# JuliaReinforcementLearning/ReinforcementLearning.jl

Measured on NVIDIA H100. Metric: env-steps/sec at 65536 CartPole envs (full PPO iteration: rollout T=32 + GAE + 4 epochs x 4 minibatches), higher is better.
Workload: dtype f32

## Files before the change

### include/b200rl.h

```cpp
#ifndef B200RL_H
#define B200RL_H

#include <stddef.h>
#include <stdint.h>

#ifdef __cplusplus
extern "C" {
#endif

typedef enum {
    B200RL_OK = 0,
    B200RL_ERR_INVALID = -1,
    B200RL_ERR_CUDA = -2,
    B200RL_ERR_UNSUPPORTED = -3,
    B200RL_ERR_ACTION = -4,
    B200RL_ERR_NCCL = -5,
    B200RL_ERR_OOM = -6
} b200rl_status;

typedef struct b200rl_ctx b200rl_ctx;
typedef struct b200rl_env b200rl_env;
typedef struct b200rl_traj b200rl_traj;
typedef struct b200rl_net b200rl_net;

// ... 68 lines not shown
int b200rl_env_reset(b200rl_env* env, int force_all);
int b200rl_env_step(b200rl_env* env, const void* actions, int actions_on_device, int auto_reset);
int b200rl_env_step_random(b200rl_env* env, int auto_reset);
int b200rl_env_get(b200rl_env* env, int field, void* host_dst, size_t bytes);
int b200rl_env_set(b200rl_env* env, int field, const void* host_src, size_t bytes);
int b200rl_env_ptr(b200rl_env* env, int field, void** dptr_out);
int b200rl_env_check(b200rl_env* env);
int b200rl_env_episode_stats(b200rl_env* env, double* out4, int reset_after);

int b200rl_gae_f32(b200rl_ctx* ctx, float* adv, const float* rewards, const float* values,
                   const uint8_t* terminal, float gamma, float lambda, int64_t R, int64_t C,
                   int dims, int on_device);
int b200rl_gae_f64(b200rl_ctx* ctx, double* adv, const double* rewards, const double* values,
                   const uint8_t* terminal, double gamma, double lambda, int64_t R, int64_t C,
                   int dims, int on_device);
int b200rl_discount_rewards_f32(b200rl_ctx* ctx, float* out, const float* rewards,
                                const uint8_t* terminal, const float* init, float gamma,
                                int64_t R, int64_t C, int dims, int on_device);
int b200rl_discount_rewards_f64(b200rl_ctx* ctx, double* out, const double* rewards,
                                const uint8_t* terminal, const double* init, double gamma,
                                int64_t R, int64_t C, int dims, int on_device);
int b200rl_discount_rewards_reduced_f32(b200rl_ctx* ctx, float* out, const float* rewards,
                                        const uint8_t* terminal, const float* init, float gamma,
                                        int64_t R, int64_t C, int dims, int on_device);
int b200rl_discount_rewards_reduced_f64(b200rl_ctx* ctx, double* out, const double* rewards,
                                        const uint8_t* terminal, const double* init, double gamma,
                                        int64_t R, int64_t C, int dims, int on_device);

int b200rl_traj_create(b200rl_ctx* ctx, int ns, int64_t lanes, int64_t capacity, int prioritized, float default_priority,
                       const uint64_t* sampler_rng, int64_t batch_size, b200rl_traj** out);
int b200rl_traj_destroy(b200rl_traj* traj);
int b200rl_traj_length(b200rl_traj* traj, int64_t* frames_out);
int b200rl_traj_lane_lengths(b200rl_traj* traj, int64_t* lengths_out);
int b200rl_traj_n_sampleable(b200rl_traj* traj, int64_t* out);
int b200rl_traj_push_state(b200rl_traj* traj, const float* obs, int on_device);
int b200rl_traj_push_episode_start(b200rl_traj* traj, const float* obs, int on_device, int mode);
int b200rl_traj_push(b200rl_traj* traj, const int32_t* action, const float* reward, const uint8_t* terminal, const float* next_obs,
                     int on_device);
int b200rl_traj_push_env(b200rl_traj* traj, b200rl_env* env, int first_state_only);
int b200rl_traj_field_bytes(b200rl_traj* traj, int field, size_t* bytes_out);
int b200rl_traj_get(b200rl_traj* traj, int field, void* host_dst, size_t bytes);
int b200rl_traj_set(b200rl_traj* traj, int field, const void* host_src, size_t bytes);
int b200rl_traj_sample(b200rl_traj* traj, float beta);
int b200rl_traj_set_nstep(b200rl_traj* traj, int32_t n, float gamma);
int b200rl_traj_batch_get(b200rl_traj* traj, int field, void* host_dst, size_t bytes);
int b200rl_traj_update_priority(b200rl_traj* traj, const float* priority, int on_device);
int b200rl_traj_total_priority(b200rl_traj* traj, float* out);

typedef struct { int32_t n_in, hidden, act, n_out, kind; } b200rl_net_desc;
int b200rl_net_nparams(const b200rl_net_desc* desc, int64_t* out);
int b200rl_net_create(b200rl_ctx* ctx, const b200rl_net_desc* desc, const float* params_host, b200rl_net** out);
int b200rl_net_destroy(b200rl_net* net);
int b200rl_net_configure_optimizer(b200rl_net* net, float lr, float beta1, float beta2, float eps, float max_grad_norm);
int b200rl_net_get(b200rl_net* net, int which, float* host_dst, int64_t count);
int b200rl_net_set(b200rl_net* net, int which, const float* host_src, int64_t count);
int b200rl_net_ptr(b200rl_net* net, int which, void** dptr_out);
int b200rl_net_get_step(b200rl_net* net, int64_t* out);
int b200rl_net_set_step(b200rl_net* net, int64_t step);
int b200rl_net_target_sync(b200rl_net* net, float rho);
int b200rl_net_act(b200rl_net* net, const float* obs, int64_t n, uint64_t* rng_dev, void* action_out, float* logp_out, float* value_out,
                   float* heads_out, int on_device);
int b200rl_net_values(b200rl_net* net, const float* obs, int64_t n, float* out, int use_target, int on_device);
int b200rl_net_q_act(b200rl_net* net, const float* obs_dev, int64_t n, uint64_t* rng_dev, float epsilon, int32_t* action_out_dev);
typedef struct {
    double eps_stable, eps_init;
    int64_t warmup_steps, decay_steps;
    int64_t step;
    int32_t kind;
    int32_t is_break_tie;
    double beta;
} b200rl_explorer;
int b200rl_net_q_explore(b200rl_net* net, const float* obs_dev, int64_t n, uint64_t* rng_dev, const b200rl_explorer* explorer,
                         int32_t* action_out_dev);
int b200rl_net_act_greedy(b200rl_net* net, const float* obs, int64_t n, void* action_out, int on_device);

typedef struct { int32_t mode, n_steps, max_episodes; } b200rl_eval_config;
int b200rl_evaluate(b200rl_net* net, b200rl_env* env, const b200rl_eval_config* cfg, uint64_t* policy_rng_dev,
                    float* returns_out, int32_t* lengths_out, int32_t* counts_out, int on_device);
int b200rl_evaluate_explore(b200rl_net* net, b200rl_env* env, int32_t n_steps, int32_t max_episodes, b200rl_explorer* ex,
                            uint64_t* explorer_rng_dev, float* returns_out, int32_t* lengths_out, int32_t* counts_out, int on_device);

typedef struct {
    float gamma, lambda, clip_range, max_grad_norm, w_actor, w_critic, w_entropy;
    float lr, beta1, beta2, eps;
    float min_sigma, max_sigma;
    int32_t normalize_advantage, n_epochs, n_microbatches, update_freq;
    int32_t algo;
} b200rl_onpolicy_config;
typedef struct b200rl_onpolicy b200rl_onpolicy;
int b200rl_net_ac_step(b200rl_net* net, const b200rl_onpolicy_config* cfg, const float* states, const void* actions,
                       const float* logp_old, const float* adv, const float* ret, int64_t total, const int32_t* idx, int64_t batch,
                       float adv_mean, float adv_inv_std, int apply_update, float* losses_out);
int b200rl_onpolicy_create(b200rl_ctx* ctx, b200rl_net* net, b200rl_env* env, const b200rl_onpolicy_config* cfg,
                           const uint64_t* policy_rng, b200rl_onpolicy** out);
int b200rl_onpolicy_destroy(b200rl_onpolicy* agent);
int b200rl_onpolicy_plan(b200rl_onpolicy* agent, void* actions_host);
int b200rl_onpolicy_act(b200rl_onpolicy* agent);
int b200rl_onpolicy_push(b200rl_onpolicy* agent);
int b200rl_onpolicy_collect(b200rl_onpolicy* agent, int n_steps);
int b200rl_onpolicy_fill(b200rl_onpolicy* agent, int* t_out, int* T_out);
int b200rl_onpolicy_update(b200rl_onpolicy* agent, const int32_t* perm_host, float* stats_host);
int b200rl_onpolicy_iterate(b200rl_onpolicy* agent, int n_iters, float* stats_host);
int b200rl_onpolicy_graph_active(b200rl_onpolicy* agent, int* out);
int b200rl_onpolicy_get(b200rl_onpolicy* agent, int field, void* host_dst, size_t bytes);
int b200rl_onpolicy_set(b200rl_onpolicy* agent, int field, const void* host_src, size_t bytes);
int b200rl_onpolicy_export_state(b200rl_onpolicy* agent, int64_t* counters3_out);
// ... 37 lines not shown
```

### reinforcementlearning.jl_b200/_lib.py

```python
import ctypes as C
import os

import numpy as np

HERE = os.path.dirname(os.path.abspath(__file__))
SO_PATH = os.environ.get("B200RL_LIB") or os.path.join(HERE, "libb200rl.so")

OK = 0
ERR_INVALID, ERR_CUDA, ERR_UNSUPPORTED, ERR_ACTION, ERR_NCCL, ERR_OOM = -1, -2, -3, -4, -5, -6

ENV_CARTPOLE, ENV_PENDULUM, ENV_MOUNTAINCAR, ENV_CARTPOLE_CONTINUOUS, ENV_MOUNTAINCAR_CONTINUOUS, ENV_ACROBOT = 0, 1, 2, 3, 4, 5
F32, F64 = 0, 1
FIELD_STATE, FIELD_OBS, FIELD_REWARD, FIELD_TERMINAL, FIELD_T, FIELD_RNG, FIELD_FLAGS, FIELD_ACTION, FIELD_EPISODE_RETURN, FIELD_EPISODE_STATS = range(10)


class B200RLError(RuntimeError):
    def __init__(self, status, msg):
        super().__init__(f"b200rl status {status}: {msg}")
        self.status = status


class CartPoleParams(C.Structure):
    _fields_ = [(n, C.c_double) for n in ("gravity", "masscart", "masspole", "totalmass", "halflength", "polemasslength",
                                          "forcemag", "dt", "thetathreshold", "xthreshold")] + [("max_steps", C.c_int64)]
# ... 56 lines not shown
    "b200rl_timer_stop_ms": (_i32, [_vp, C.POINTER(_f32)]),
    "b200rl_timer_record": (_i32, [_vp, _i32]),
    "b200rl_timer_elapsed_ms": (_i32, [_vp, _i32, _i32, C.POINTER(_f32)]),
    "b200rl_debug_phase_slots": (_i32, [_vp, _i32]),
    "b200rl_malloc": (_i32, [_vp, _sz, _pp]),
    "b200rl_free": (_i32, [_vp, _vp]),
    "b200rl_host_alloc": (_i32, [_vp, _sz, _pp]),
    "b200rl_host_free": (_i32, [_vp, _vp]),
    "b200rl_memcpy_h2d": (_i32, [_vp, _vp, _vp, _sz, _i32]),
    "b200rl_memcpy_d2h": (_i32, [_vp, _vp, _vp, _sz, _i32]),
    "b200rl_memset": (_i32, [_vp, _vp, _i32, _sz]),
    "b200rl_flush_l2": (_i32, [_vp]),
    "b200rl_launch_count": (_i32, [_vp, C.POINTER(_u64)]),
    "b200rl_env_create": (_i32, [_vp, _i32, _i32, _i64, _vp, _vp, _pp]),
    "b200rl_env_destroy": (_i32, [_vp]),
    "b200rl_env_set_max_timeout": (_i32, [_vp, _i64]),
    "b200rl_env_copy": (_i32, [_vp, _pp]),
    "b200rl_env_seed": (_i32, [_vp, _vp]),
    "b200rl_env_reset": (_i32, [_vp, _i32]),
    "b200rl_env_step": (_i32, [_vp, _vp, _i32, _i32]),
    "b200rl_env_step_random": (_i32, [_vp, _i32]),
    "b200rl_env_get": (_i32, [_vp, _i32, _vp, _sz]),
    "b200rl_env_set": (_i32, [_vp, _i32, _vp, _sz]),
    "b200rl_env_ptr": (_i32, [_vp, _i32, _pp]),
    "b200rl_env_check": (_i32, [_vp]),
    "b200rl_env_episode_stats": (_i32, [_vp, _vp, _i32]),
    "b200rl_gae_f32": (_i32, [_vp, _vp, _vp, _vp, _vp, _f32, _f32, _i64, _i64, _i32, _i32]),
    "b200rl_gae_f64": (_i32, [_vp, _vp, _vp, _vp, _vp, _f64, _f64, _i64, _i64, _i32, _i32]),
    "b200rl_discount_rewards_f32": (_i32, [_vp, _vp, _vp, _vp, _vp, _f32, _i64, _i64, _i32, _i32]),
    "b200rl_discount_rewards_f64": (_i32, [_vp, _vp, _vp, _vp, _vp, _f64, _i64, _i64, _i32, _i32]),
    "b200rl_discount_rewards_reduced_f32": (_i32, [_vp, _vp, _vp, _vp, _vp, _f32, _i64, _i64, _i32, _i32]),
    "b200rl_discount_rewards_reduced_f64": (_i32, [_vp, _vp, _vp, _vp, _vp, _f64, _i64, _i64, _i32, _i32]),
    "b200rl_traj_create": (_i32, [_vp, _i32, _i64, _i64, _i32, _f32, _vp, _i64, _pp]),
    "b200rl_traj_destroy": (_i32, [_vp]),
    "b200rl_traj_length": (_i32, [_vp, C.POINTER(_i64)]),
    "b200rl_traj_lane_lengths": (_i32, [_vp, _vp]),
    "b200rl_traj_n_sampleable": (_i32, [_vp, C.POINTER(_i64)]),
    "b200rl_traj_push_episode_start": (_i32, [_vp, _vp, _i32, _i32]),
    "b200rl_traj_field_bytes": (_i32, [_vp, _i32, C.POINTER(_sz)]),
    "b200rl_traj_get": (_i32, [_vp, _i32, _vp, _sz]),
    "b200rl_traj_set": (_i32, [_vp, _i32, _vp, _sz]),
    "b200rl_traj_push_state": (_i32, [_vp, _vp, _i32]),
    "b200rl_traj_push": (_i32, [_vp, _vp, _vp, _vp, _vp, _i32]),
    "b200rl_traj_push_env": (_i32, [_vp, _vp, _i32]),
    "b200rl_traj_sample": (_i32, [_vp, _f32]),
    "b200rl_traj_set_nstep": (_i32, [_vp, _i32, _f32]),
    "b200rl_traj_batch_get": (_i32, [_vp, _i32, _vp, _sz]),
    "b200rl_traj_update_priority": (_i32, [_vp, _vp, _i32]),
    "b200rl_traj_total_priority": (_i32, [_vp, C.POINTER(_f32)]),
    "b200rl_net_nparams": (_i32, [_vp, C.POINTER(_i64)]),
    "b200rl_net_create": (_i32, [_vp, _vp, _vp, _pp]),
    "b200rl_net_destroy": (_i32, [_vp]),
    "b200rl_net_configure_optimizer": (_i32, [_vp, _f32, _f32, _f32, _f32, _f32]),
    "b200rl_net_get": (_i32, [_vp, _i32, _vp, _i64]),
    "b200rl_net_set": (_i32, [_vp, _i32, _vp, _i64]),
    "b200rl_net_ptr": (_i32, [_vp, _i32, _pp]),
    "b200rl_net_get_step": (_i32, [_vp, C.POINTER(_i64)]),
    "b200rl_net_set_step": (_i32, [_vp, _i64]),
    "b200rl_net_target_sync": (_i32, [_vp, _f32]),
    "b200rl_net_act": (_i32, [_vp, _vp, _i64, _vp, _vp, _vp, _vp, _vp, _i32]),
    "b200rl_net_values": (_i32, [_vp, _vp, _i64, _vp, _i32, _i32]),
    "b200rl_net_q_act": (_i32, [_vp, _vp, _i64, _vp, _f32, _vp]),
    "b200rl_net_q_explore": (_i32, [_vp, _vp, _i64, _vp, _vp, _vp]),
    "b200rl_net_act_greedy": (_i32, [_vp, _vp, _i64, _vp, _i32]),
    "b200rl_evaluate": (_i32, [_vp, _vp, _vp, _vp, _vp, _vp, _vp, _i32]),
    "b200rl_evaluate_explore": (_i32, [_vp, _vp, _i32, _i32, _vp, _vp, _vp, _vp, _vp, _i32]),
    "b200rl_net_ac_step": (_i32, [_vp, _vp, _vp, _vp, _vp, _vp, _vp, _i64, _vp, _i64, _f32, _f32, _i32, _vp]),
    "b200rl_onpolicy_create": (_i32, [_vp, _vp, _vp, _vp, _vp, _pp]),
    "b200rl_onpolicy_destroy": (_i32, [_vp]),
    "b200rl_onpolicy_plan": (_i32, [_vp, _vp]),
    "b200rl_onpolicy_act": (_i32, [_vp]),
    "b200rl_onpolicy_push": (_i32, [_vp]),
    "b200rl_onpolicy_collect": (_i32, [_vp, _i32]),
    "b200rl_onpolicy_fill": (_i32, [_vp, C.POINTER(_i32), C.POINTER(_i32)]),
    "b200rl_onpolicy_update": (_i32, [_vp, _vp, _vp]),
    "b200rl_onpolicy_iterate": (_i32, [_vp, _i32, _vp]),
    "b200rl_onpolicy_graph_active": (_i32, [_vp, C.POINTER(_i32)]),
    "b200rl_onpolicy_get": (_i32, [_vp, _i32, _vp, _sz]),
    "b200rl_onpolicy_set": (_i32, [_vp, _i32, _vp, _sz]),
    "b200rl_onpolicy_export_state": (_i32, [_vp, _vp]),
    "b200rl_onpolicy_import_state": (_i32, [_vp, _vp]),
    "b200rl_onpolicy_time_kernel": (_i32, [_vp, _i32, _i32, C.POINTER(_f32)]),
    "b200rl_dqn_update": (_i32, [_vp, _vp, _vp, _vp]),
    "b200rl_dqn_last_td": (_i32, [_vp, _vp, _vp, _i64]),
    "b200rl_replay_create": (_i32, [_vp, _vp, _vp, _vp, _vp, _pp]),
    "b200rl_replay_run": (_i32, [_vp, _vp, _vp, _vp, _i64, _vp]),
    "b200rl_replay_graph_active": (_i32, [_vp, C.POINTER(_i32)]),
    "b200rl_replay_destroy": (_i32, [_vp]),
    "b200rl_set_tensor_cores": (_i32, [_i32]),
    "b200rl_set_fused_step": (_i32, [_i32]),
    "b200rl_comm_unique_id": (_i32, [_vp]),
    "b200rl_comm_init": (_i32, [_vp, _i32, _i32, _vp]),
    "b200rl_comm_allreduce_f32": (_i32, [_vp, _vp, _i64]),
    "b200rl_comm_p2p_export": (_i32, [_vp, _vp, _pp]),
    "b200rl_comm_p2p_open": (_i32, [_vp, _vp, _pp]),
    "b200rl_comm_p2p_attach": (_i32, [_vp, _vp]),
    "b200rl_ctx_pci_bus_id": (_i32, [_vp, _vp, _i32]),
    "b200rl_comm_p2p_set_exclusive": (_i32, [_vp, _i32]),
}

_LIB = None


def load():
    global _LIB
    if _LIB is not None:
# ... 113 lines not shown
```

### reinforcementlearning.jl_b200/csrc/algo.cu

```cuda
#include <map>

#include "greedy.cuh"
#include "internal.h"
#include "nn.cuh"
#include "replay_schedule.h"
#include "ring.cuh"

static void* env_field(b200rl_env* e, int f) { void* p = nullptr; b200rl_env_ptr(e, f, &p); return p; }

namespace {
__global__ void clamp_copy_kernel(float* __restrict__ dst, const float* __restrict__ src, int64_t n, float lo, float hi) {
    int64_t i = (int64_t)blockIdx.x * blockDim.x + threadIdx.x;
    if (i < n) dst[i] = fminf(fmaxf(src[i], lo), hi);
}
__global__ void greedy_select_kernel(const float* __restrict__ heads, MlpDesc d, int64_t n, int clamp, float lo, float hi,
                                     uint32_t* __restrict__ out) {
    int64_t i = (int64_t)blockIdx.x * blockDim.x + threadIdx.x;
    if (i >= n) return;
    float z[kOutMax];
#pragma unroll
    for (int o = 0; o < kOutMax; ++o) z[o] = o < d.nout ? heads[(int64_t)d.nout * i + o] : 0.f;
    uint32_t a = greedy::greedy_action(d, z);
    if (clamp) a = __float_as_uint(fminf(fmaxf(__uint_as_float(a), lo), hi));
    out[i] = a;
// ... 267 lines not shown
extern "C" {

int b200rl_net_nparams(const b200rl_net_desc* d, int64_t* out) {
    MlpDesc a, c;
    TRY(make_descs(d, &a, &c));
    REQUIRE(out, B200RL_ERR_INVALID, "null out");
    *out = is_q_kind(d->kind) ? a.nparams() : a.nparams() + c.nparams();
    return B200RL_OK;
}

int b200rl_net_destroy(b200rl_net* n) {
    if (!n) return B200RL_OK;
    cudaSetDevice(n->ctx->device);
    cudaStreamSynchronize(n->ctx->stream);
    cudaFree(n->params); cudaFree(n->grad); cudaFree(n->m); cudaFree(n->v); cudaFree(n->beta_t); cudaFree(n->target);
    cudaFree(n->partial); cudaFree(n->loss_partial); cudaFree(n->loss4); cudaFree(n->gnorm); cudaFree(n->cta_sumsq); cudaFree(n->counters);
    delete n;
    return B200RL_OK;
}

int b200rl_net_create(b200rl_ctx* ctx, const b200rl_net_desc* d, const float* params_host, b200rl_net** out) {
    TRY(ctx_bind(ctx));
    REQUIRE(out && params_host, B200RL_ERR_INVALID, "null argument");
    b200rl_net* n = new b200rl_net();
    memset(n, 0, sizeof *n);
    n->ctx = ctx; n->kind = d ? d->kind : 0;
    int s = make_descs(d, &n->actor, &n->critic);
    if (s != B200RL_OK) { delete n; return s; }
    n->np = is_q_kind(n->kind) ? n->actor.nparams() : n->actor.nparams() + n->critic.nparams();
    n->lr = 1e-3f; n->b1 = 0.9f; n->b2 = 0.999f; n->eps = 1e-8f; n->max_grad_norm = 0.5f;
    size_t bytes = (size_t)n->np * sizeof(float);
    n->n_partials = is_q_kind(n->kind) ? nn_dqn_max_partials(ctx, n->actor.H) : nn_grid_ctas(ctx, n->actor.H);
    int n_loss_rows = 2 * (n->n_partials > ctx->sm_count ? n->n_partials : ctx->sm_count);
#define NET_TRY(x) CUDA_TRY_OR(x, b200rl_net_destroy(n))
    NET_TRY(cudaMalloc(&n->params, bytes)); NET_TRY(cudaMalloc(&n->grad, bytes)); NET_TRY(cudaMalloc(&n->m, bytes)); NET_TRY(cudaMalloc(&n->v, bytes));
    NET_TRY(cudaMalloc(&n->beta_t, 2 * sizeof(float)));
    if (is_q_kind(n->kind)) NET_TRY(cudaMalloc(&n->target, bytes));
    NET_TRY(cudaMalloc(&n->partial, (size_t)n->n_partials * bytes));
    NET_TRY(cudaMalloc(&n->loss_partial, (size_t)n_loss_rows * 4 * sizeof(float)));
    NET_TRY(cudaMalloc(&n->loss4, 4 * sizeof(float))); NET_TRY(cudaMalloc(&n->gnorm, sizeof(float)));
    NET_TRY(cudaMalloc(&n->cta_sumsq, 256 * sizeof(double))); NET_TRY(cudaMalloc(&n->counters, 4 * sizeof(unsigned int)));
    NET_TRY(cudaMemsetAsync(n->counters, 0, 4 * sizeof(unsigned int), ctx->stream));
    NET_TRY(cudaMemcpyAsync(n->params, params_host, bytes, cudaMemcpyHostToDevice, ctx->stream));
    if (is_q_kind(n->kind)) NET_TRY(cudaMemcpyAsync(n->target, params_host, bytes, cudaMemcpyHostToDevice, ctx->stream));
    NET_TRY(cudaMemsetAsync(n->grad, 0, bytes, ctx->stream)); NET_TRY(cudaMemsetAsync(n->m, 0, bytes, ctx->stream));
    NET_TRY(cudaMemsetAsync(n->v, 0, bytes, ctx->stream));
    NET_TRY(cudaMemsetAsync(n->partial, 0, (size_t)n->n_partials * bytes, ctx->stream));
    NET_TRY(cudaMemsetAsync(n->loss_partial, 0, (size_t)n_loss_rows * 4 * sizeof(float), ctx->stream));
    float bt[2] = {n->b1, n->b2};
    NET_TRY(cudaMemcpyAsync(n->beta_t, bt, sizeof bt, cudaMemcpyHostToDevice, ctx->stream));
    NET_TRY(cudaStreamSynchronize(ctx->stream));
#undef NET_TRY
    *out = n;
    return B200RL_OK;
}

int b200rl_net_configure_optimizer(b200rl_net* n, float lr, float beta1, float beta2, float eps, float max_grad_norm) {
    REQUIRE(n, B200RL_ERR_INVALID, "null net");
    TRY(ctx_bind(n->ctx));
    n->lr = lr; n->b1 = beta1; n->b2 = beta2; n->eps = eps; n->max_grad_norm = max_grad_norm;
    if (n->n_updates == 0) {
        float bt[2] = {beta1, beta2};
        CUDA_TRY(cudaMemcpyAsync(n->beta_t, bt, sizeof bt, cudaMemcpyHostToDevice, n->ctx->stream));
        CUDA_TRY(cudaStreamSynchronize(n->ctx->stream));
    }
    return B200RL_OK;
}

static int net_buf(b200rl_net* n, int which, float** p, int64_t* len) {
    switch (which) {
        case 0: *p = n->params; *len = n->np; return B200RL_OK;
        case 1: *p = n->grad; *len = n->np; return B200RL_OK;
        case 2: *p = n->m; *len = n->np; return B200RL_OK;
        case 3: *p = n->v; *len = n->np; return B200RL_OK;
        case 4: *p = n->beta_t; *len = 2; return B200RL_OK;
        case 5: REQUIRE(n->target, B200RL_ERR_INVALID, "no target network"); *p = n->target; *len = n->np; return B200RL_OK;
    }
    REQUIRE(false, B200RL_ERR_INVALID, "unknown buffer id");
}
int b200rl_net_get(b200rl_net* n, int which, float* host_dst, int64_t count) {
    REQUIRE(n && host_dst, B200RL_ERR_INVALID, "null argument");
    TRY(ctx_bind(n->ctx));
    float* p; int64_t len;
    TRY(net_buf(n, which, &p, &len));
    REQUIRE(count >= len, B200RL_ERR_INVALID, "destination too small");
    CUDA_TRY(cudaMemcpyAsync(host_dst, p, (size_t)len * 4, cudaMemcpyDeviceToHost, n->ctx->stream));
    CUDA_TRY(cudaStreamSynchronize(n->ctx->stream));
    return B200RL_OK;
}
int b200rl_net_set(b200rl_net* n, int which, const float* host_src, int64_t count) {
    REQUIRE(n && host_src, B200RL_ERR_INVALID, "null argument");
    TRY(ctx_bind(n->ctx));
    float* p; int64_t len;
    TRY(net_buf(n, which, &p, &len));
    REQUIRE(count >= len, B200RL_ERR_INVALID, "source too small");
    CUDA_TRY(cudaMemcpyAsync(p, host_src, (size_t)len * 4, cudaMemcpyHostToDevice, n->ctx->stream));
    CUDA_TRY(cudaStreamSynchronize(n->ctx->stream));
    return B200RL_OK;
}
int b200rl_net_ptr(b200rl_net* n, int which, void** dptr_out) {
    REQUIRE(n && dptr_out, B200RL_ERR_INVALID, "null argument");
    float* p; int64_t len;
    TRY(net_buf(n, which, &p, &len));
    *dptr_out = p;
    return B200RL_OK;
}
// ... 907 lines not shown
```

### reinforcementlearning.jl_b200/csrc/nn_tc.cu

```cuda
#include "nn.cuh"
#include "perm.cuh"
#include "policy.cuh"
#include "tc_fwd.cuh"
#include "tc_split.h"
#include "wgmma.cuh"

namespace {

using tcfwd::G_F;
using tcfwd::GW_S;
using tcfwd::WIMG_BYTES;
using tcfwd::split2;
using tcfwd::wimg_off;
constexpr int TM = tcfwd::TM;
constexpr int H = tcfwd::H;
constexpr float kScaleW = tcfwd::kScale;

constexpr int NT7 = 512;
constexpr int kMaxStage = 10;
constexpr int GF_T = 128;
constexpr int GS_T = 16 * GF_T;
constexpr int FIMG = 8 * GS_T;
constexpr float kScaleH = 64.0f, kScaleX = 64.0f;
constexpr int kNo = 2;

struct SmemBwd {
    static_assert(FIMG % 128 == 0 && WIMG_BYTES % 128 == 0 && (2 * GS_T) % 16 == 0, "operand images must stay 128-byte aligned");
    alignas(128) uint8_t FP_full[FIMG];
    alignas(128) uint8_t FP_lo[FIMG];
    alignas(128) uint8_t FH_lo[FIMG];
    alignas(128) uint8_t FH_full[FIMG];
    alignas(16) uint8_t FH_ones[2 * GS_T];
    alignas(128) uint8_t FQ_full[FIMG];
    alignas(128) uint8_t FQ_lo[FIMG];
    alignas(128) uint8_t B1[WIMG_BYTES];
    alignas(128) uint8_t XT[2][2 * GS_T];
    alignas(128) uint8_t AH_full[FIMG];
    alignas(128) uint8_t AH_lo[FIMG];
    alignas(16) float D[TM * H];
    float W1[kInMax * H];
    float b1[H], b2[H];
    float W3[H * kNo];
    float b3[kNo];
    float Zp[4 * kNo * TM];
    float Red[32];
    double RedD[16];
    float step_scale;
    alignas(8) uint64_t bar1;
    alignas(8) uint64_t bar2;
    alignas(8) uint64_t bar3;
    alignas(8) uint64_t bar4;
    float AccW2[64 * 65 + 64];
    float AccD4[64 * 9];
};
__device__ __forceinline__ int d_off(int s, int col) { return s * H + ((((col >> 2) ^ (s & 15))) << 2) + (col & 3); }
__device__ __forceinline__ void d_ld16(const float* D, int s, int f0, float (&v)[16]) {
#pragma unroll
    for (int u = 0; u < 4; ++u) {
        const float4 q4 = *reinterpret_cast<const float4*>(D + d_off(s, f0 + 4 * u));
        v[4 * u] = q4.x; v[4 * u + 1] = q4.y; v[4 * u + 2] = q4.z; v[4 * u + 3] = q4.w;
    }
}
template <int TB>
__device__ __forceinline__ void gemm_ts3(float (&d)[32], const uint8_t* a_hi, const uint8_t* a_lo, int h, uint64_t dB, uint32_t b_step) {
    const uint64_t dA = wg::make_desc(wg::smem_u32(a_hi) + 8 * h * GF_T, GS_T, GF_T), dAl = wg::make_desc(wg::smem_u32(a_lo) + 8 * h * GF_T, GS_T, GF_T);
    wg::fence();
#pragma unroll
    for (int k = 0; k < 4; ++k) {
        const uint32_t aa = k * 2 * GS_T, bb = k * b_step;
        wg::mma_m64n64k16<0, TB>(d, wg::desc_add(dA, aa), wg::desc_add(dB, bb), k ? 1u : 0u);
        wg::mma_m64n64k16<0, TB>(d, wg::desc_add(dA, aa), wg::desc_add(dB, 8 * GW_S + bb), 1u);
        wg::mma_m64n64k16<0, TB>(d, wg::desc_add(dAl, aa), wg::desc_add(dB, bb), 1u);
    }
    wg::commit();
    wg::wait_all();
}
__device__ __forceinline__ uint32_t fimg_off(int f, int s) { return (uint32_t)((f >> 3) * GS_T + (s >> 3) * GF_T + (s & 7) * 16 + (f & 7) * 2); }
__device__ __forceinline__ void store16_feat(uint8_t* img, int f0, int s, const uint32_t (&v)[8]) {
    uint8_t* p = img + fimg_off(f0, s);
    *reinterpret_cast<uint4*>(p) = make_uint4(v[0], v[1], v[2], v[3]);
    *reinterpret_cast<uint4*>(p + GS_T) = make_uint4(v[4], v[5], v[6], v[7]);
}
using b200perm::perm_index;
using b200perm::perm_index_bits;

__device__ __forceinline__ float lane_transpose_reduce32(float (&v)[32], int lane) {
#pragma unroll
    for (int st = 0; st < 5; ++st) {
        const int half = 16 >> st, off = 16 >> st;
        const bool upper = (lane & off) != 0;
#pragma unroll
        for (int n = 0; n < half; ++n) {
            float send = upper ? v[n] : v[n + half];
            float keep = upper ? v[n + half] : v[n];
            v[n] = keep + __shfl_xor_sync(0xffffffffu, send, off);
        }
    }
    return v[0];
}

__device__ __forceinline__ void worker_sync() { asm volatile("bar.sync 1, 512;" ::: "memory"); }
__device__ __forceinline__ void group_sync(int q) { asm volatile("bar.sync %0, 128;" ::"r"(5 + q) : "memory"); }
__device__ __forceinline__ void ready_arrive(int id) { asm volatile("bar.arrive %0, 640;" ::"r"(id) : "memory"); }
__device__ __forceinline__ void ready_wait(int id) { asm volatile("bar.sync %0, 640;" ::"r"(id) : "memory"); }
#ifdef B200RL_K7_TIMING
__device__ unsigned long long g_k7_phase[40];
__device__ int g_k7_watch = 0;
#define K7_T(i) do { if (tid == (g_k7_watch & 0xFFFF) && (int)blockIdx.x == (g_k7_watch >> 16)) { long long now_ = clock64(); g_k7_phase[i] += (unsigned long long)(now_ - tprev_); tprev_ = now_; } } while (0)
#else
#define K7_T(i) do { } while (0)
#endif
constexpr int NT7_ALL = NT7 + 128;
constexpr int kRegsMma = 64, kRegsWorker = 104;
static_assert(128 * kRegsMma + NT7 * kRegsWorker <= NT7_ALL * 96, "setmaxnreg split must fit the CTA's register allocation");
constexpr int kBarRdyA = 2, kBarRdyB = 3, kBarRdyC = 4;

template <int ACT>
__global__ void __launch_bounds__(NT7_ALL, 1)
ac_loss_grad_tc_kernel(MlpDesc actor, MlpDesc critic, const float* params , AcHyper hp, AcBatch b, float* partial,
                       float* __restrict__ loss_partial, int64_t np_total, float scale_base ,
                       OptStep st ,
                       int n_actor ) {
    extern __shared__ __align__(1024) unsigned char smem_raw[];
    SmemBwd& sm = *reinterpret_cast<SmemBwd*>(smem_raw);
    const int role = (int)blockIdx.x < n_actor ? 0 : 1;
    const int cta = role ? (int)blockIdx.x - n_actor : (int)blockIdx.x;
    const int nctas = role ? (int)gridDim.x - n_actor : n_actor;
    const int nrows = max(n_actor, (int)gridDim.x - n_actor);
    const float scale_p = scale_base * (role ? 4.0f : 64.0f);
    const MlpDesc d = role ? critic : actor;
    const int act = ACT >= 0 ? ACT : d.act;
    const bool relu = act == B200RL_ACT_RELU;
    const int64_t poff = role ? actor.nparams() : 0;
    const float* __restrict__ p = params + poff;
    const int tid = threadIdx.x, warp = tid >> 5, lane = tid & 31;
    const int q = warp & 3, c = (warp >> 2) & 3;
    const int s = 32 * q + lane;
    {
        const float* b1 = p + (int64_t)H * d.in;
        const float* W2 = b1 + H;
        const float* b2 = W2 + (int64_t)H * H;
        const float s1 = relu ? kScaleH : 1.0f;
        for (int k = tid; k < kInMax * H; k += NT7_ALL) sm.W1[k] = (k / H) < d.in ? p[k] * s1 : 0.f;
        for (int k = tid; k < H; k += NT7_ALL) { sm.b1[k] = b1[k] * s1; sm.b2[k] = b2[k]; }
        for (int k = tid; k < H * kNo; k += NT7_ALL) {
            int j = k / kNo, o = k % kNo;
            sm.W3[k] = o < d.nout ? p[head_w<false>(d, o, j)] : 0.f;
        }
        if (tid < kNo) sm.b3[tid] = tid < d.nout ? p[head_b<false>(d, tid)] : 0.f;
        tcfwd::fill_w2_image<NT7_ALL>(sm.B1, W2);
    }
    for (int k = tid; k < 2 * TM; k += NT7_ALL)
        *reinterpret_cast<uint4*>(sm.FH_ones + 16 * k) = make_uint4(k < TM ? 0x3C00u : 0u, 0u, 0u, 0u);
    if (tid == 32) {
        wg::mbar_init(&sm.bar1, 128); wg::mbar_init(&sm.bar2, 128); wg::mbar_init(&sm.bar3, 128); wg::mbar_init(&sm.bar4, 128);
    }
    wg::fence_proxy_async();
    __syncthreads();
    const float inv_s1 = 1.0f / (kScaleH * kScaleW), inv_s3 = 1.0f / (scale_p * kScaleH), inv_sp = 1.0f / scale_p, inv_s4 = 1.0f / (scale_p * kScaleX);
    const int64_t ntiles = (b.B + TM - 1) / TM;

    if (warp >= NT7 / 32) {
        asm volatile("setmaxnreg.dec.sync.aligned.u32 %0;" ::"n"(kRegsMma));
        const int t = tid - NT7, row0 = 16 * (t >> 5) + ((t & 31) >> 2), col0 = 2 * (t & 3);
        const uint64_t dB1k = wg::make_desc(wg::smem_u32(sm.B1), G_F, GW_S);
        const uint64_t dB1t = wg::make_desc(wg::smem_u32(sm.B1), GW_S, G_F);
        float dacc[32];
        auto store_d = [&](int h) {
#pragma unroll
            for (int j = 0; j < 8; ++j)
#pragma unroll
                for (int hh = 0; hh < 2; ++hh)
                    *reinterpret_cast<float2*>(sm.D + d_off(64 * h + row0 + 8 * hh, 8 * j + col0)) = make_float2(dacc[4 * j + 2 * hh], dacc[4 * j + 2 * hh + 1]);
        };
        auto gemm1 = [&](int h) { gemm_ts3<0>(dacc, sm.AH_full, sm.AH_lo, h, dB1k, 2 * G_F); };
        auto gemm2 = [&](int h) { gemm_ts3<1>(dacc, sm.FP_full, sm.FP_lo, h, dB1t, 2 * GW_S); };
        auto gemm3 = [&]() {
            const uint64_t dPh = wg::make_desc(wg::smem_u32(sm.FP_full), GF_T, GS_T), dPl = wg::make_desc(wg::smem_u32(sm.FP_lo), GF_T, GS_T);
            const uint64_t dHh = wg::make_desc(wg::smem_u32(sm.FH_full), GF_T, GS_T), dHl = wg::make_desc(wg::smem_u32(sm.FH_lo), GF_T, GS_T);
            wg::fence();
#pragma unroll
            for (int k = 0; k < 8; ++k) {
                const uint32_t a = k * 2 * GF_T;
                wg::mma_m64n64k16<1, 1>(dacc, wg::desc_add(dPh, a), wg::desc_add(dHh, a), k ? 1u : 0u);
                wg::mma_m64n64k16<1, 1>(dacc, wg::desc_add(dPl, a), wg::desc_add(dHh, a), 1u);
                wg::mma_m64n64k16<1, 1>(dacc, wg::desc_add(dPh, a), wg::desc_add(dHl, a), 1u);
            }
            wg::commit();
            wg::wait_all();
#pragma unroll
            for (int j = 0; j < 8; ++j)
#pragma unroll
                for (int hh = 0; hh < 2; ++hh)
#pragma unroll
                    for (int e = 0; e < 2; ++e) sm.AccW2[(row0 + 8 * hh) * 65 + 8 * j + col0 + e] += dacc[4 * j + 2 * hh + e];
            const uint64_t dOnes = wg::make_desc(wg::smem_u32(sm.FH_ones), GF_T, GS_T);
            float d8[4] = {0.f, 0.f, 0.f, 0.f};
            wg::fence();
#pragma unroll
            for (int k = 0; k < 8; ++k) {
                const uint32_t a = k * 2 * GF_T;
                wg::mma_m64n8k16<1, 1>(d8, wg::desc_add(dPh, a), wg::desc_add(dOnes, a), k ? 1u : 0u);
                wg::mma_m64n8k16<1, 1>(d8, wg::desc_add(dPl, a), wg::desc_add(dOnes, a), 1u);
            }
            wg::commit();
            wg::wait_all();
            if (col0 == 0) {
                sm.AccW2[64 * 65 + row0] += d8[0];
                sm.AccW2[64 * 65 + row0 + 8] += d8[2];
            }
        };
        auto gemm4 = [&](int buf) {
            const uint64_t dQh = wg::make_desc(wg::smem_u32(sm.FQ_full), GF_T, GS_T), dQl = wg::make_desc(wg::smem_u32(sm.FQ_lo), GF_T, GS_T);
            const uint64_t dX = wg::make_desc(wg::smem_u32(sm.XT[buf]), GF_T, GS_T);
            float d4[4] = {0.f, 0.f, 0.f, 0.f};
            wg::fence();
#pragma unroll
            for (int k = 0; k < 8; ++k) {
                const uint32_t a = k * 2 * GF_T;
                wg::mma_m64n8k16<1, 1>(d4, wg::desc_add(dQh, a), wg::desc_add(dX, a), k ? 1u : 0u);
                wg::mma_m64n8k16<1, 1>(d4, wg::desc_add(dQh, a), wg::desc_add(dX, GS_T + a), 1u);
                wg::mma_m64n8k16<1, 1>(d4, wg::desc_add(dQl, a), wg::desc_add(dX, a), 1u);
            }
            wg::commit();
            wg::wait_all();
#pragma unroll
            for (int hh = 0; hh < 2; ++hh)
#pragma unroll
                for (int e = 0; e < 2; ++e)
                    if (col0 + e < 5) sm.AccD4[(row0 + 8 * hh) * 9 + col0 + e] += d4[2 * hh + e];
        };
        if (cta < ntiles) {
            ready_wait(kBarRdyB);
            for (int h = 0; h < 2; ++h) { gemm1(h); store_d(h); }
            wg::mbar_arrive(&sm.bar1);
        }
        int buf = 0;
        for (int64_t tile = cta; tile < ntiles; tile += nctas, buf ^= 1) {
            const bool has_next = tile + nctas < ntiles;
            ready_wait(kBarRdyA);
            for (int h = 0; h < 2; ++h) { gemm2(h); store_d(h); }
            wg::mbar_arrive(&sm.bar2);
            gemm3();
            wg::mbar_arrive(&sm.bar3);
            if (has_next) {
                ready_wait(kBarRdyB);
                gemm1(0);
            }
            ready_wait(kBarRdyC);
            if (has_next) {
                store_d(0);
                gemm1(1);
                store_d(1);
                wg::mbar_arrive(&sm.bar1);
            }
            gemm4(buf);
            wg::mbar_arrive(&sm.bar4);
        }
    } else {
    asm volatile("setmaxnreg.inc.sync.aligned.u32 %0;" ::"n"(kRegsWorker));
    float g3[2][16];
    float gb3a0 = 0.f, gb3a1 = 0.f;
#pragma unroll
    for (int k = 0; k < 16; ++k) { g3[0][k] = 0.f; g3[1][k] = 0.f; }
    float l0 = 0.f, l1 = 0.f;
    float mean = 0.f, inv_std = 1.f;
    if (hp.normalize_adv && b.norm2) { mean = b.norm2[0]; inv_std = b.norm2[1]; }
    uint32_t ph1 = 0, ph2 = 0, ph3 = 0, ph4 = 0;
    bool gemm4_pending = false;
    int xbuf = 0;
#ifdef B200RL_K7_TIMING
    long long tprev_ = clock64();
#endif
    const int pbits = b200perm::perm_bits(b.perm_n);
    const uint32_t pkey = ac_perm_key(b);
    auto index_of = [&](int64_t t) -> int32_t {
        const int64_t j = t * TM + s;
        if (t >= ntiles || j >= b.B) return -1;
        return b.idx ? b.idx[j] : (int32_t)perm_index_bits((uint32_t)(b.perm_offset + j), b.perm_n, pkey, pbits);
    };
    auto request = [&](int32_t g, float (&x)[kInMax], float (&a)[4]) {
#pragma unroll
        for (int k = 0; k < kInMax; ++k) { x[k] = 0.f; a[k] = 0.f; }
        if (g < 0) return;
        if (b.rec) {
            const float4 v0 = b.rec[2 * (int64_t)g], v1 = b.rec[2 * (int64_t)g + 1];
            x[0] = v0.x; x[1] = v0.y; x[2] = v0.z; x[3] = v0.w;
            a[0] = v1.x; a[1] = v1.y; a[2] = v1.z; a[3] = v1.w;
        } else {
#pragma unroll
            for (int i = 0; i < kInMax; ++i)
                if (i < b.ns) x[i] = b.states[(int64_t)b.ns * g + i];
            a[0] = reinterpret_cast<const float*>(b.actions)[g];
            a[1] = b.logp_old ? b.logp_old[g] : 0.f;
            a[2] = b.adv[g];
            a[3] = b.ret[g];
        }
    };
    float pfx[kInMax] = {0.f, 0.f, 0.f, 0.f}, pfa[4] = {0.f, 0.f, 0.f, 0.f};
    float aux[4] = {0.f, 0.f, 0.f, 0.f};
    int32_t gi_next = -1;
    bool gemm3_pending = false;
    float* const out = partial + (int64_t)cta * np_total + poff;
    float* const gW1 = out;
    float* const gb1 = out + (int64_t)H * d.in;
    float* const gW2 = gb1 + H;
    float* const gb2 = gW2 + (int64_t)H * H;
    for (int k = tid; k < 64 * 65 + 64; k += NT7) sm.AccW2[k] = 0.f;
    for (int k = tid; k < 64 * 9; k += NT7) sm.AccD4[k] = 0.f;
    float xo[kInMax];
    auto publish = [&](int64_t t) {
#pragma unroll
        for (int i = 0; i < kInMax; ++i) xo[i] = pfx[i];
        aux[0] = pfa[0];
        aux[1] = role == 0 ? pfa[1] : 0.f;
        aux[2] = role == 0 ? (hp.normalize_adv ? (pfa[2] - mean) * inv_std : pfa[2]) : 0.f;
        aux[3] = role == 0 ? 0.f : pfa[3];
        if (c == 0) {
            uint32_t h01, l01, h23, l23;
            split2(xo[0] * kScaleX, xo[1] * kScaleX, h01, l01);
            split2(xo[2] * kScaleX, xo[3] * kScaleX, h23, l23);
            uint8_t* xt = sm.XT[xbuf] + fimg_off(0, s);
            *reinterpret_cast<uint4*>(xt) = make_uint4(h01, h23, 0x3C00u, 0u);
            *reinterpret_cast<uint4*>(xt + GS_T) = make_uint4(l01, l23, 0u, 0u);
        }
        K7_T(16);
        xbuf ^= 1;
        request(gi_next, pfx, pfa);
        gi_next = index_of(t + 2 * nctas);
        K7_T(17);
    };
    uint32_t h1pos = 0, h1pos_tile = 0;
    auto layer1 = [&]() {
        uint32_t pos = 0;
        uint32_t hi8[8], lo8[8];
#pragma unroll
        for (int ch = 0; ch < 4; ++ch) {
            const int f0 = 16 * c + 4 * ch;
            float4 bb = *reinterpret_cast<const float4*>(sm.b1 + f0);
            float h[4] = {bb.x, bb.y, bb.z, bb.w};
#pragma unroll
            for (int k = 0; k < kInMax; ++k) {
                float4 w = *reinterpret_cast<const float4*>(sm.W1 + k * H + f0);
                h[0] = fmaf(w.x, xo[k], h[0]); h[1] = fmaf(w.y, xo[k], h[1]); h[2] = fmaf(w.z, xo[k], h[2]); h[3] = fmaf(w.w, xo[k], h[3]);
            }
            if (relu) {
#pragma unroll
                for (int e = 0; e < 4; ++e) { pos |= (h[e] > 0.f ? 1u : 0u) << (4 * ch + e); h[e] = fmaxf(h[e], 0.f); }
            } else {
#pragma unroll
                for (int e = 0; e < 4; ++e) h[e] = act_f(act, h[e]) * kScaleH;
            }
            split2(h[0], h[1], hi8[2 * ch], lo8[2 * ch]);
            split2(h[2], h[3], hi8[2 * ch + 1], lo8[2 * ch + 1]);
        }
        h1pos = pos;
        store16_feat(sm.AH_full, 16 * c, s, hi8);
        store16_feat(sm.AH_lo, 16 * c, s, lo8);
    };
    if (cta < ntiles) {
        request(index_of(cta), pfx, pfa);
        gi_next = index_of(cta + nctas);
        publish(cta);
        layer1();
        wg::fence_proxy_async();
        ready_arrive(kBarRdyB);
    }
#ifdef B200RL_K7_TIMING
    tprev_ = clock64();
#endif
    for (int64_t tile = cta; tile < ntiles; tile += nctas) {
        const bool has_next = tile + nctas < ntiles;
        wg::mbar_wait(&sm.bar1, ph1);
        ph1 ^= 1u;
        K7_T(0);
        float h2[16];
        {
            float v[16];
            d_ld16(sm.D, s, 16 * c, v);
            float zp[kNo] = {0.f, 0.f};
#pragma unroll
            for (int k = 0; k < 16; ++k) {
                const int f = 16 * c + k;
                h2[k] = act_f(act, fmaf(v[k], inv_s1, sm.b2[f]));
                float2 w = *reinterpret_cast<const float2*>(sm.W3 + f * kNo);
                zp[0] = fmaf(w.x, h2[k], zp[0]); zp[1] = fmaf(w.y, h2[k], zp[1]);
            }
#pragma unroll
            for (int o = 0; o < kNo; ++o) sm.Zp[(c * kNo + o) * TM + s] = zp[o];
        }
        K7_T(1);
        group_sync(q);
        K7_T(2);
        {
            float z[kNo];
#pragma unroll
            for (int o = 0; o < kNo; ++o)
                z[o] = sm.b3[o] + ((sm.Zp[o * TM + s] + sm.Zp[(kNo + o) * TM + s]) + (sm.Zp[(2 * kNo + o) * TM + s] + sm.Zp[(3 * kNo + o) * TM + s]));
            const bool valid = (tile * TM + s) < b.B;
            const policy::LossOut<kNo> lo_ = policy::sample_loss(actor.heads2, actor.nout, role, hp, b.inv_B, z, aux[0], aux[1], aux[2], aux[3]);
            float dz[kNo];
#pragma unroll
            for (int o = 0; o < kNo; ++o) dz[o] = valid ? lo_.dz[o] : 0.f;
            if (c == 0 && valid) { l0 += lo_.l0; l1 += lo_.l1; gb3a0 += dz[0]; gb3a1 += dz[1]; }
            const float dzs0 = dz[0] * scale_p, dzs1 = dz[1] * scale_p;
            float dp[16];
#pragma unroll
            for (int k = 0; k < 16; ++k) {
                const int f = 16 * c + k;
                float2 w = *reinterpret_cast<const float2*>(sm.W3 + f * kNo);
                const float dh = fmaf(w.x, dzs0, w.y * dzs1);
                dp[k] = relu ? (h2[k] > 0.f ? dh : 0.f) : dh * (1.f - h2[k] * h2[k]);
                g3[0][k] = fmaf(dz[0], h2[k], g3[0][k]);
                g3[1][k] = fmaf(dz[1], h2[k], g3[1][k]);
            }
            uint32_t hi8[8], lo8[8];
#pragma unroll
            for (int m = 0; m < 8; ++m) split2(dp[2 * m], dp[2 * m + 1], hi8[m], lo8[m]);
            K7_T(3);
            if (gemm3_pending) {
                wg::mbar_wait(&sm.bar3, ph3);
                ph3 ^= 1u;
                gemm3_pending = false;
            }
            K7_T(4);
            store16_feat(sm.FP_full, 16 * c, s, hi8);
            store16_feat(sm.FP_lo, 16 * c, s, lo8);
            {
                const uint32_t off = fimg_off(16 * c, s);
                const uint4 h0 = *reinterpret_cast<const uint4*>(sm.AH_full + off), h1 = *reinterpret_cast<const uint4*>(sm.AH_full + off + GS_T);
                const uint4 l0 = *reinterpret_cast<const uint4*>(sm.AH_lo + off), l1 = *reinterpret_cast<const uint4*>(sm.AH_lo + off + GS_T);
                *reinterpret_cast<uint4*>(sm.FH_full + off) = h0; *reinterpret_cast<uint4*>(sm.FH_full + off + GS_T) = h1;
                *reinterpret_cast<uint4*>(sm.FH_lo + off) = l0; *reinterpret_cast<uint4*>(sm.FH_lo + off + GS_T) = l1;
            }
        }
        K7_T(5);
        wg::fence_proxy_async();
        ready_arrive(kBarRdyA);
        gemm3_pending = true;
        K7_T(6);
        K7_T(7);
        h1pos_tile = h1pos;
        if (has_next) {
            if (gemm4_pending) {
                wg::mbar_wait(&sm.bar4, ph4);
                ph4 ^= 1u;
                gemm4_pending = false;
            }
            publish(tile + nctas);
            K7_T(8);
            K7_T(9);
            layer1();
            wg::fence_proxy_async();
            K7_T(10);
            ready_arrive(kBarRdyB);
            K7_T(11);
        }
        K7_T(12);
        wg::mbar_wait(&sm.bar2, ph2);
        ph2 ^= 1u;
        K7_T(13);
        {
            float v[16];
            d_ld16(sm.D, s, 16 * c, v);
#pragma unroll
            for (int k = 0; k < 16; ++k) v[k] *= 1.0f / kScaleW;
            if (relu) {
#pragma unroll
                for (int k = 0; k < 16; ++k) v[k] = ((h1pos_tile >> k) & 1u) ? v[k] : 0.f;
            } else {
                const float inv_h = 1.0f / kScaleH;
#pragma unroll
                for (int g8 = 0; g8 < 2; ++g8) {
                    const uint32_t off = fimg_off(16 * c + 8 * g8, s);
                    const uint4 hv = *reinterpret_cast<const uint4*>(sm.FH_full + off), lv = *reinterpret_cast<const uint4*>(sm.FH_lo + off);
                    const uint32_t hw[4] = {hv.x, hv.y, hv.z, hv.w}, lw[4] = {lv.x, lv.y, lv.z, lv.w};
#pragma unroll
                    for (int m = 0; m < 4; ++m) {
                        const float2 hf = __half22float2(*reinterpret_cast<const __half2*>(&hw[m])), lf = __half22float2(*reinterpret_cast<const __half2*>(&lw[m]));
                        v[8 * g8 + 2 * m] *= dact_f(act, (hf.x + lf.x) * inv_h);
                        v[8 * g8 + 2 * m + 1] *= dact_f(act, (hf.y + lf.y) * inv_h);
                    }
                }
            }
            if (gemm4_pending) {
                wg::mbar_wait(&sm.bar4, ph4);
                ph4 ^= 1u;
                gemm4_pending = false;
            }
            {
                uint32_t hi8[8], lo8[8];
#pragma unroll
                for (int m = 0; m < 8; ++m) split2(v[2 * m], v[2 * m + 1], hi8[m], lo8[m]);
                store16_feat(sm.FQ_full, 16 * c, s, hi8);
                store16_feat(sm.FQ_lo, 16 * c, s, lo8);
            }
            gemm4_pending = true;
        }
        K7_T(14);
#ifdef B200RL_K7_TIMING
        if (tid == (g_k7_watch & 0xFFFF) && (int)blockIdx.x == (g_k7_watch >> 16)) g_k7_phase[15] += 1;
#endif
        wg::fence_proxy_async();
        ready_arrive(kBarRdyC);
    }
    if (gemm3_pending) wg::mbar_wait(&sm.bar3, ph3);
    if (gemm4_pending) wg::mbar_wait(&sm.bar4, ph4);
    worker_sync();
    for (int k = tid; k < H * H; k += NT7) gW2[k] = sm.AccW2[(k & 63) * 65 + (k >> 6)] * inv_s3;
    if (tid < H) {
        gb2[tid] = sm.AccW2[64 * 65 + tid] * inv_sp;
        gb1[tid] = sm.AccD4[tid * 9 + 4] * inv_sp;
        for (int i = 0; i < d.in; ++i) gW1[tid + H * i] = sm.AccD4[tid * 9 + i] * inv_s4;
    }
    if (cta >= (int)gridDim.x - nctas) {
        const int64_t ooff = role ? 0 : actor.nparams(), on = role ? actor.nparams() : critic.nparams();
        float* orow = partial + (int64_t)cta * np_total + ooff;
        for (int64_t kk = tid; kk < on; kk += NT7) orow[kk] = 0.f;
    }
    float* red = reinterpret_cast<float*>(sm.FP_full);
    static_assert(offsetof(SmemBwd, XT) - offsetof(SmemBwd, FP_full) >= (2 * TM * 65 + 2 * 8 * 64) * 4, "drain scratch");
    {
        constexpr int RS = 65;
        float* seg = red + 2 * TM * RS;
#pragma unroll
        for (int k = 0; k < 16; ++k) {
            red[0 * TM * RS + s * RS + 16 * c + k] = g3[0][k];
            red[1 * TM * RS + s * RS + 16 * c + k] = g3[1][k];
        }
        worker_sync();
        {
            const int col = tid & 63, g = tid >> 6;
#pragma unroll
            for (int m = 0; m < 2; ++m) {
                float a = 0.f;
#pragma unroll
                for (int ss = 0; ss < 16; ++ss) a += red[m * TM * RS + (16 * g + ss) * RS + col];
                seg[(m * 8 + g) * 64 + col] = a;
            }
        }
        worker_sync();
        if (tid < 2 * H) {
            const int m = tid >> 6, col = tid & 63;
            float a = 0.f;
#pragma unroll
            for (int g = 0; g < 8; ++g) a += seg[(m * 8 + g) * 64 + col];
            if (m < d.nout) out[head_w<false>(d, m, col)] = a;
        }
        worker_sync();
    }
    if (c == 0) { red[s] = gb3a0; red[TM + s] = gb3a1; }
    worker_sync();
    if (warp < d.nout) {
        float a = (red[warp * TM + lane] + red[warp * TM + 32 + lane]) + (red[warp * TM + 64 + lane] + red[warp * TM + 96 + lane]);
#pragma unroll
        for (int o = 16; o > 0; o >>= 1) a += __shfl_xor_sync(0xffffffffu, a, o);
        if (lane == 0) out[head_b<false>(d, warp)] = a;
// ... 185 lines not shown
```

Measured before the change: 279.3 million.

## Move dP1 epilogue into MMA warpgroup and reschedule backward pipeline stages

The MMA warpgroup now applies the layer-1 activation derivative itself (using ReLU masks that the workers store in shared memory, double-buffered) and writes the FQ operand straight from its accumulators. This removes the worker round-trip through the D buffer, the bar2 mbarrier and the kBarRdyC handshake. The order is also changed so gemm1 for the next tile is issued before gemm3, and the bias-gradient MMA reuses the X tile rather than a dedicated ones image. A separate API to set the critic activation is added. The risk is that the MMA warpgroup becomes longer on the critical path and that the new named barrier and the buffer-parity handling carry correctness hazards.

Result: faster. 310.2 million (median of 6 runs) (+11.1%).

```diff
diff --git a/include/b200rl.h b/include/b200rl.h
--- a/include/b200rl.h
+++ b/include/b200rl.h
@@ -144,6 +144,7 @@
 int b200rl_net_create(b200rl_ctx* ctx, const b200rl_net_desc* desc, const float* params_host, b200rl_net** out);
 int b200rl_net_destroy(b200rl_net* net);
 int b200rl_net_configure_optimizer(b200rl_net* net, float lr, float beta1, float beta2, float eps, float max_grad_norm);
+int b200rl_net_set_critic_act(b200rl_net* net, int act);
 int b200rl_net_get(b200rl_net* net, int which, float* host_dst, int64_t count);
 int b200rl_net_set(b200rl_net* net, int which, const float* host_src, int64_t count);
 int b200rl_net_ptr(b200rl_net* net, int which, void** dptr_out);
diff --git a/reinforcementlearning.jl_b200/_lib.py b/reinforcementlearning.jl_b200/_lib.py
--- a/reinforcementlearning.jl_b200/_lib.py
+++ b/reinforcementlearning.jl_b200/_lib.py
@@ -132,6 +132,7 @@
     "b200rl_net_create": (_i32, [_vp, _vp, _vp, _pp]),
     "b200rl_net_destroy": (_i32, [_vp]),
     "b200rl_net_configure_optimizer": (_i32, [_vp, _f32, _f32, _f32, _f32, _f32]),
+    "b200rl_net_set_critic_act": (_i32, [_vp, _i32]),
     "b200rl_net_get": (_i32, [_vp, _i32, _vp, _i64]),
     "b200rl_net_set": (_i32, [_vp, _i32, _vp, _i64]),
     "b200rl_net_ptr": (_i32, [_vp, _i32, _pp]),
diff --git a/reinforcementlearning.jl_b200/csrc/algo.cu b/reinforcementlearning.jl_b200/csrc/algo.cu
--- a/reinforcementlearning.jl_b200/csrc/algo.cu
+++ b/reinforcementlearning.jl_b200/csrc/algo.cu
@@ -343,6 +343,14 @@
     NET_TRY(cudaStreamSynchronize(ctx->stream));
 #undef NET_TRY
     *out = n;
+    return B200RL_OK;
+}
+
+int b200rl_net_set_critic_act(b200rl_net* n, int act) {
+    REQUIRE(n, B200RL_ERR_INVALID, "null net");
+    REQUIRE(!is_q_kind(n->kind), B200RL_ERR_INVALID, "only actor-critic networks have a critic trunk");
+    REQUIRE(act == 0 || act == 1, B200RL_ERR_INVALID, "act must be 0 (relu) or 1 (tanh)");
+    n->critic.act = act;
     return B200RL_OK;
 }
 
diff --git a/reinforcementlearning.jl_b200/csrc/nn_tc.cu b/reinforcementlearning.jl_b200/csrc/nn_tc.cu
--- a/reinforcementlearning.jl_b200/csrc/nn_tc.cu
+++ b/reinforcementlearning.jl_b200/csrc/nn_tc.cu
@@ -30,7 +30,6 @@
     alignas(128) uint8_t FP_lo[FIMG];
     alignas(128) uint8_t FH_lo[FIMG];
     alignas(128) uint8_t FH_full[FIMG];
-    alignas(16) uint8_t FH_ones[2 * GS_T];
     alignas(128) uint8_t FQ_full[FIMG];
     alignas(128) uint8_t FQ_lo[FIMG];
     alignas(128) uint8_t B1[WIMG_BYTES];
@@ -38,6 +37,7 @@
     alignas(128) uint8_t AH_full[FIMG];
     alignas(128) uint8_t AH_lo[FIMG];
     alignas(16) float D[TM * H];
+    uint64_t H1pos[2][TM];
     float W1[kInMax * H];
     float b1[H], b2[H];
     float W3[H * kNo];
@@ -47,7 +47,6 @@
     double RedD[16];
     float step_scale;
     alignas(8) uint64_t bar1;
-    alignas(8) uint64_t bar2;
     alignas(8) uint64_t bar3;
     alignas(8) uint64_t bar4;
     float AccW2[64 * 65 + 64];
@@ -113,7 +112,9 @@
 constexpr int NT7_ALL = NT7 + 128;
 constexpr int kRegsMma = 64, kRegsWorker = 104;
 static_assert(128 * kRegsMma + NT7 * kRegsWorker <= NT7_ALL * 96, "setmaxnreg split must fit the CTA's register allocation");
-constexpr int kBarRdyA = 2, kBarRdyB = 3, kBarRdyC = 4;
+constexpr int kBarRdyA = 2, kBarRdyB = 3;
+constexpr int kBarMma = 4;
+__device__ __forceinline__ void mma_sync() { asm volatile("bar.sync %0, 128;" ::"n"(kBarMma) : "memory"); }
 
 template <int ACT>
 __global__ void __launch_bounds__(NT7_ALL, 1)
@@ -150,10 +151,8 @@
         if (tid < kNo) sm.b3[tid] = tid < d.nout ? p[head_b<false>(d, tid)] : 0.f;
         tcfwd::fill_w2_image<NT7_ALL>(sm.B1, W2);
     }
-    for (int k = tid; k < 2 * TM; k += NT7_ALL)
-        *reinterpret_cast<uint4*>(sm.FH_ones + 16 * k) = make_uint4(k < TM ? 0x3C00u : 0u, 0u, 0u, 0u);
     if (tid == 32) {
-        wg::mbar_init(&sm.bar1, 128); wg::mbar_init(&sm.bar2, 128); wg::mbar_init(&sm.bar3, 128); wg::mbar_init(&sm.bar4, 128);
+        wg::mbar_init(&sm.bar1, 128); wg::mbar_init(&sm.bar3, 128); wg::mbar_init(&sm.bar4, 128);
     }
     wg::fence_proxy_async();
     __syncthreads();
@@ -175,7 +174,33 @@
         };
         auto gemm1 = [&](int h) { gemm_ts3<0>(dacc, sm.AH_full, sm.AH_lo, h, dB1k, 2 * G_F); };
         auto gemm2 = [&](int h) { gemm_ts3<1>(dacc, sm.FP_full, sm.FP_lo, h, dB1t, 2 * GW_S); };
-        auto gemm3 = [&]() {
+        auto store_dp1 = [&](int h, int pbuf) {
+#pragma unroll
+            for (int hh = 0; hh < 2; ++hh) {
+                const int ss = 64 * h + row0 + 8 * hh;
+                const uint64_t pos = relu ? sm.H1pos[pbuf][ss] >> col0 : 0u;
+#pragma unroll
+                for (int j = 0; j < 8; ++j) {
+                    const uint32_t off = fimg_off(8 * j + col0, ss);
+                    float v0 = dacc[4 * j + 2 * hh] * (1.0f / kScaleW), v1 = dacc[4 * j + 2 * hh + 1] * (1.0f / kScaleW);
+                    if (relu) {
+                        v0 = ((pos >> (8 * j)) & 1u) ? v0 : 0.f;
+                        v1 = ((pos >> (8 * j + 1)) & 1u) ? v1 : 0.f;
+                    } else {
+                        const float inv_h = 1.0f / kScaleH;
+                        const float2 hf = __half22float2(*reinterpret_cast<const __half2*>(sm.FH_full + off));
+                        const float2 lf = __half22float2(*reinterpret_cast<const __half2*>(sm.FH_lo + off));
+                        v0 *= dact_f(act, (hf.x + lf.x) * inv_h);
+                        v1 *= dact_f(act, (hf.y + lf.y) * inv_h);
+                    }
+                    uint32_t hi, lo;
+                    split2(v0, v1, hi, lo);
+                    *reinterpret_cast<uint32_t*>(sm.FQ_full + off) = hi;
+                    *reinterpret_cast<uint32_t*>(sm.FQ_lo + off) = lo;
+                }
+            }
+        };
+        auto gemm3 = [&](int buf) {
             const uint64_t dPh = wg::make_desc(wg::smem_u32(sm.FP_full), GF_T, GS_T), dPl = wg::make_desc(wg::smem_u32(sm.FP_lo), GF_T, GS_T);
             const uint64_t dHh = wg::make_desc(wg::smem_u32(sm.FH_full), GF_T, GS_T), dHl = wg::make_desc(wg::smem_u32(sm.FH_lo), GF_T, GS_T);
             wg::fence();
@@ -194,18 +219,18 @@
                 for (int hh = 0; hh < 2; ++hh)
 #pragma unroll
                     for (int e = 0; e < 2; ++e) sm.AccW2[(row0 + 8 * hh) * 65 + 8 * j + col0 + e] += dacc[4 * j + 2 * hh + e];
-            const uint64_t dOnes = wg::make_desc(wg::smem_u32(sm.FH_ones), GF_T, GS_T);
+            const uint64_t dX = wg::make_desc(wg::smem_u32(sm.XT[buf]), GF_T, GS_T);
             float d8[4] = {0.f, 0.f, 0.f, 0.f};
             wg::fence();
 #pragma unroll
             for (int k = 0; k < 8; ++k) {
                 const uint32_t a = k * 2 * GF_T;
-                wg::mma_m64n8k16<1, 1>(d8, wg::desc_add(dPh, a), wg::desc_add(dOnes, a), k ? 1u : 0u);
-                wg::mma_m64n8k16<1, 1>(d8, wg::desc_add(dPl, a), wg::desc_add(dOnes, a), 1u);
+                wg::mma_m64n8k16<1, 1>(d8, wg::desc_add(dPh, a), wg::desc_add(dX, a), k ? 1u : 0u);
+                wg::mma_m64n8k16<1, 1>(d8, wg::desc_add(dPl, a), wg::desc_add(dX, a), 1u);
             }
             wg::commit();
             wg::wait_all();
-            if (col0 == 0) {
+            if (col0 == 4) {
                 sm.AccW2[64 * 65 + row0] += d8[0];
                 sm.AccW2[64 * 65 + row0 + 8] += d8[2];
             }
@@ -237,23 +262,17 @@
         }
         int buf = 0;
         for (int64_t tile = cta; tile < ntiles; tile += nctas, buf ^= 1) {
-            const bool has_next = tile + nctas < ntiles;
             ready_wait(kBarRdyA);
-            for (int h = 0; h < 2; ++h) { gemm2(h); store_d(h); }
-            wg::mbar_arrive(&sm.bar2);
-            gemm3();
+            for (int h = 0; h < 2; ++h) { gemm2(h); store_dp1(h, buf); }
+            wg::fence_proxy_async();
+            if (tile + nctas < ntiles) {
+                ready_wait(kBarRdyB);
+                for (int h = 0; h < 2; ++h) { gemm1(h); store_d(h); }
+                wg::mbar_arrive(&sm.bar1);
+            }
+            gemm3(buf);
             wg::mbar_arrive(&sm.bar3);
-            if (has_next) {
-                ready_wait(kBarRdyB);
-                gemm1(0);
-            }
-            ready_wait(kBarRdyC);
-            if (has_next) {
-                store_d(0);
-                gemm1(1);
-                store_d(1);
-                wg::mbar_arrive(&sm.bar1);
-            }
+            mma_sync();
             gemm4(buf);
             wg::mbar_arrive(&sm.bar4);
         }
@@ -266,9 +285,10 @@
     float l0 = 0.f, l1 = 0.f;
     float mean = 0.f, inv_std = 1.f;
     if (hp.normalize_adv && b.norm2) { mean = b.norm2[0]; inv_std = b.norm2[1]; }
-    uint32_t ph1 = 0, ph2 = 0, ph3 = 0, ph4 = 0;
+    uint32_t ph1 = 0, ph3 = 0, ph4 = 0;
     bool gemm4_pending = false;
     int xbuf = 0;
+    int pbuf = 0;
 #ifdef B200RL_K7_TIMING
     long long tprev_ = clock64();
 #endif
@@ -330,7 +350,6 @@
         gi_next = index_of(t + 2 * nctas);
         K7_T(17);
     };
-    uint32_t h1pos = 0, h1pos_tile = 0;
     auto layer1 = [&]() {
         uint32_t pos = 0;
         uint32_t hi8[8], lo8[8];
@@ -354,7 +373,8 @@
             split2(h[0], h[1], hi8[2 * ch], lo8[2 * ch]);
             split2(h[2], h[3], hi8[2 * ch + 1], lo8[2 * ch + 1]);
         }
-        h1pos = pos;
+        if (relu) reinterpret_cast<uint16_t*>(&sm.H1pos[pbuf][s])[c] = (uint16_t)pos;
+        pbuf ^= 1;
         store16_feat(sm.AH_full, 16 * c, s, hi8);
         store16_feat(sm.AH_lo, 16 * c, s, lo8);
     };
@@ -436,73 +456,26 @@
         }
         K7_T(5);
         wg::fence_proxy_async();
+        if (gemm4_pending) {
+            wg::mbar_wait(&sm.bar4, ph4);
+            ph4 ^= 1u;
+        }
+        K7_T(6);
         ready_arrive(kBarRdyA);
         gemm3_pending = true;
-        K7_T(6);
+        gemm4_pending = true;
         K7_T(7);
-        h1pos_tile = h1pos;
         if (has_next) {
-            if (gemm4_pending) {
-                wg::mbar_wait(&sm.bar4, ph4);
-                ph4 ^= 1u;
-                gemm4_pending = false;
-            }
             publish(tile + nctas);
-            K7_T(8);
-            K7_T(9);
             layer1();
             wg::fence_proxy_async();
-            K7_T(10);
+            K7_T(8);
             ready_arrive(kBarRdyB);
-            K7_T(11);
-        }
-        K7_T(12);
-        wg::mbar_wait(&sm.bar2, ph2);
-        ph2 ^= 1u;
-        K7_T(13);
-        {
-            float v[16];
-            d_ld16(sm.D, s, 16 * c, v);
-#pragma unroll
-            for (int k = 0; k < 16; ++k) v[k] *= 1.0f / kScaleW;
-            if (relu) {
-#pragma unroll
-                for (int k = 0; k < 16; ++k) v[k] = ((h1pos_tile >> k) & 1u) ? v[k] : 0.f;
-            } else {
-                const float inv_h = 1.0f / kScaleH;
-#pragma unroll
-                for (int g8 = 0; g8 < 2; ++g8) {
-                    const uint32_t off = fimg_off(16 * c + 8 * g8, s);
-                    const uint4 hv = *reinterpret_cast<const uint4*>(sm.FH_full + off), lv = *reinterpret_cast<const uint4*>(sm.FH_lo + off);
-                    const uint32_t hw[4] = {hv.x, hv.y, hv.z, hv.w}, lw[4] = {lv.x, lv.y, lv.z, lv.w};
-#pragma unroll
-                    for (int m = 0; m < 4; ++m) {
-                        const float2 hf = __half22float2(*reinterpret_cast<const __half2*>(&hw[m])), lf = __half22float2(*reinterpret_cast<const __half2*>(&lw[m]));
-                        v[8 * g8 + 2 * m] *= dact_f(act, (hf.x + lf.x) * inv_h);
-                        v[8 * g8 + 2 * m + 1] *= dact_f(act, (hf.y + lf.y) * inv_h);
-                    }
-                }
-            }
-            if (gemm4_pending) {
-                wg::mbar_wait(&sm.bar4, ph4);
-                ph4 ^= 1u;
-                gemm4_pending = false;
-            }
-            {
-                uint32_t hi8[8], lo8[8];
-#pragma unroll
-                for (int m = 0; m < 8; ++m) split2(v[2 * m], v[2 * m + 1], hi8[m], lo8[m]);
-                store16_feat(sm.FQ_full, 16 * c, s, hi8);
-                store16_feat(sm.FQ_lo, 16 * c, s, lo8);
-            }
-            gemm4_pending = true;
-        }
-        K7_T(14);
+            K7_T(9);
+        }
 #ifdef B200RL_K7_TIMING
         if (tid == (g_k7_watch & 0xFFFF) && (int)blockIdx.x == (g_k7_watch >> 16)) g_k7_phase[15] += 1;
 #endif
-        wg::fence_proxy_async();
-        ready_arrive(kBarRdyC);
     }
     if (gemm3_pending) wg::mbar_wait(&sm.bar3, ph3);
     if (gemm4_pending) wg::mbar_wait(&sm.bar4, ph4);
```
